# KAIST-AILab/SyncVSR

Hardware: AMD Instinct MI355X
Metric: lip-clips/sec training (29x88x88) (higher is better)
Workload: dtype bf16; 1 GPU; LRW training step (fwd+bwd+allreduce+clip+AdamW), ResNet18 + 6-layer 512-d encoder + vq audio-token CE head, random-init weights, N(0,1) clips 29x88x88, uniform tokens/labels; per_gpu_batch=32, global_batch=32, parallelism=dp1, hip_graph=False, enqueue=native step list

## Files before the change

include/syncvsr_hip.h:

```cpp
#ifndef SYNCVSR_HIP_H
#define SYNCVSR_HIP_H

#include <stdint.h>

#ifndef __HIP_PLATFORM_AMD__
typedef void* hipStream_t;
#else
#include <hip/hip_runtime_api.h>
#endif

#define SVSR_OK 0
#define SVSR_ERR_ARG 1001
#define SVSR_GRAD_ADD_DW 1
#define SVSR_GRAD_ADD_DB 2
#define SVSR_ERR_GROUP_OPEN 1003
#define SVSR_ERR_NO_GROUP 1004
#define SVSR_ERR_MASK_SIZE 1005

typedef struct svsr_wgrad_problem {
    const void* x; const void* dy; float* dw; float* dbias; const int* plan_dev; const int* meta;
    int Nimg; int in_pix; int Ci; int in_pitch; int Co; int out_pix; int out_pitch; int wt_taps;
} svsr_wgrad_problem;

typedef struct svsr_enc_layer {
// ... 27 lines not shown
int svsr_rows_plan(int Nimg, int P, int src0, int dst0, int Co_out, int* words, int cap_words, int* meta);
int svsr_igemm_fwd_kgroups(const int* meta, int Ci, int Co, int bn_epilogue);
int svsr_igemm_fwd(const void* in, const void* wt, void* out, void* out_pre, const float* bias, const void* addend, float* stats, const int* plan_dev, const int* meta, int Nimg, int in_pix, int Ci, int in_pitch, int Co, int out_pix, int out_pitch, int wt_taps, int act, int out_f32, float alpha, const unsigned* drop_seed, unsigned drop_site, float drop_p, hipStream_t stream);

int svsr_wgrad_plan(int Nimg, int H, int W, int Ci, int Co, int k, int stride, int pad, int* words, int cap_words, int* meta, int64_t* part_floats);
int svsr_wgrad_rows_plan(int Nimg, int P, int src0, int dst0, int Ci, int Co, int has_bias, int* words, int cap_words, int* meta, int64_t* part_floats);
int svsr_igemm_wgrad(const void* x, const void* dyp, float* dw, float* dbias, const int* plan_dev, const int* meta, int Nimg, int in_pix, int Ci, int in_pitch, int Co, int out_pix, int out_pitch, int wt_taps, float* part, int64_t part_floats, hipStream_t stream);
int svsr_wgrad_rows_plan_tile(int Nimg, int P, int src0, int dst0, int Ci, int Co, int has_bias, int bc, int* words, int cap_words, int* meta, int64_t* part_floats);
int64_t svsr_igemm_wgrad_group_bytes(int n);
int svsr_igemm_wgrad_group(const svsr_wgrad_problem* problems, int n, void* table_dev, int64_t table_bytes, hipStream_t stream);
int svsr_igemm_wgrad_v2(const void* x, const void* dyp, float* dw, float* dbias, const int* plan_dev, const int* meta, int Nimg, int in_pix, int Ci, int in_pitch, int Co, int out_pix, int out_pitch, int wt_taps, float* part, int64_t part_floats, int mode, hipStream_t stream);
int svsr_igemm_wgrad_group_v2(const svsr_wgrad_problem* problems, const int* modes, int n, void* table_dev, int64_t table_bytes, hipStream_t stream);

int svsr_conv3x3_c64_stat_rows(int Nimg, int H, int W);
int64_t svsr_conv3x3_c64_pixtab(int Nimg, int H, int W, int* out, int64_t cap);
int svsr_conv3x3_c64(const void* in, const void* wt, void* out, const void* addend, float* stats, int Nimg, int H, int W, const int* dy, const int* dx, const int* tw, const int* pixtab, hipStream_t stream);

int svsr_igemm_dgrad_bn(const void* in, const void* wt, void* out, const void* addend, float* stats, const int* plan_dev, const int* meta, int Nimg, int in_pix, int Ci, int in_pitch, int Co, int out_pix, int out_pitch, int wt_taps, const void* y, const void* x, const float* mean, const float* rstd, const float* gamma, const float* beta, int act, hipStream_t stream);
int svsr_igemm_dgrad_relu(const void* in, const void* wt, void* out, float* stats, const int* plan_dev, const int* meta, int Nimg, int in_pix, int Ci, int in_pitch, int Co, int out_pix, int out_pitch, int wt_taps, const void* y, const float* zeros, const float* ones, float gscale, hipStream_t stream);
int svsr_igemm_dgrad2(const void* in, const void* wt, const void* in2, const void* wt2, void* out, void* out_pre, const float* bias, float* stats, const int* plan_dev, const int* meta, int Nimg, int in_pix, int Ci, int in_pitch, int Co, int out_pix, int out_pitch, int wt_taps, int act, int out_f32, float alpha, const unsigned* drop_seed, unsigned drop_site, float drop_p, hipStream_t stream);
int svsr_igemm_dgrad2_bn(const void* in, const void* wt, const void* in2, const void* wt2, void* out, float* stats, const int* plan_dev, const int* meta, int Nimg, int in_pix, int Ci, int in_pitch, int Co, int out_pix, int out_pitch, int wt_taps, const void* y, const void* x, const float* mean, const float* rstd, const float* gamma, const float* beta, int act, hipStream_t stream);
int svsr_conv3x3_c64_dgrad_bn(const void* in, const void* wt, void* out, const void* addend, float* stats, int Nimg, int H, int W, const int* dy, const int* dx, const int* tw, const void* y, const void* x, const float* mean, const float* rstd, const float* gamma, const float* beta, int act, const int* pixtab, hipStream_t stream);
int svsr_bn_bwd_from_stats(const void* g, const void* x, const float* mean, const float* rstd, const float* gamma, const float* stats, int nrows, float* coef, float* dgamma, float* dbeta, void* dx, int64_t npix, int C, hipStream_t stream);


int svsr_conv3x3_wgrad_plan(int Nimg, int H, int W, int Ci, int Co, int* splits, int64_t* part_floats);
int svsr_conv3x3_wgrad(const void* x, const void* dy, float* dw, int Nimg, int H, int W, int Ci, int Co, float* part, int64_t part_floats, hipStream_t stream);
int svsr_conv3x3_wgrad_v2(const void* x, const void* dy, float* dw, int Nimg, int H, int W, int Ci, int Co, float* part, int64_t part_floats, int mode, hipStream_t stream);
int svsr_conv3x3_wgrad_chain(const void* x, const void* dy, float* dw, int Nimg, int H, int W, int Ci, int Co, float* part, int64_t part_floats, int mode, int defer, const float* pend_part, float* pend_dw, int pend_splits, int pend_Ci, int pend_Co, int pend_mode, hipStream_t stream);
int svsr_conv3x3_wgrad_reduce(const float* part, float* dw, int splits, int Ci, int Co, int mode, hipStream_t stream);

int svsr_stem_conv_fwd_stat_rows(int B, int T, int H, int W);
int64_t svsr_stem_conv_fwd_ws_bytes(int B, int T, int H, int W);
int svsr_stem_conv_fwd(const float* vid, const float* w, void* out, float* stats, int B, int T, int H, int W, void* ws, int64_t ws_bytes, hipStream_t stream);

int svsr_stem_conv_wgrad_plan(int B, int T, int H, int W, int* splits, int64_t* part_floats);
int svsr_stem_conv_wgrad(const float* vid, const void* dy, float* dw, int B, int T, int H, int W, int use_tr, float* part, int64_t part_floats, hipStream_t stream);

int svsr_stem_bwd_wgrad_ok(int B, int T, int H, int W);
int svsr_stem_bwd_wgrad(const float* vid, const void* gpool, const void* amax, const void* x, const float* mean, const float* rstd, const float* coef, float* dw, int B, int T, int H, int W, float* part, int64_t part_floats, hipStream_t stream);

int svsr_bn_finalize(const float* part, int nrows, int C, float count, float eps, float momentum, float* mean, float* rstd, float* running_mean, float* running_var, int64_t* num_batches_tracked, hipStream_t stream);

int svsr_bn_eval_prepare(const float* running_mean, const float* running_var, int C, float eps, float* mean, float* rstd, hipStream_t stream);

int svsr_bn_act_fwd(const void* x, const void* res, void* y, const float* mean, const float* rstd, const float* gamma, const float* beta, int64_t npix, int C, int act, hipStream_t stream);

int svsr_bn_act_bwd_rows(int64_t npix, int C);
int svsr_bn_act_bwd(const void* dy, const void* y, const void* x, const float* mean, const float* rstd, const float* gamma, float* slots, float* coef, float* dgamma, float* dbeta, void* dx, void* dres, int64_t npix, int C, int act, const float* beta, const void* res, hipStream_t stream);

int svsr_stem_bn_act_pool_fwd(const void* x, void* y, void* amax, const float* mean, const float* rstd, const float* gamma, const float* beta, int N, int Hc, int Wc, int Hp, int Wp, int C, int act, void* xwin, hipStream_t stream);

int svsr_stem_bn_act_pool_bwd_rows(int N, int Hc, int Wc, int C);
int svsr_stem_bn_act_pool_bwd(const void* dpool, const void* amax, const void* x, const float* mean, const float* rstd, const float* gamma, const float* beta, float* slots, float* coef, float* dgamma, float* dbeta, void* dx, int N, int Hc, int Wc, int Hp, int Wp, int C, int act, const void* xwin, void* gpool, hipStream_t stream);

int svsr_avgpool_fwd(const void* x, void* y, int64_t N, int HW, int C, hipStream_t stream);
int svsr_avgpool_bwd(const void* dy, void* dx, int64_t N, int HW, int C, hipStream_t stream);

int svsr_add_ln_fwd(const void* a, const void* r, const float* gamma, const float* beta, void* y, float* mean, float* rstd, int R, int D, float eps, hipStream_t stream);
int svsr_add_ln_bwd_rows(int R);
int svsr_add_ln_bwd(const void* dy, const void* a, const void* r, const float* gamma, const float* mean, const float* rstd, void* ds, float* dgamma, float* dbeta, int R, int D, const void* addend, float* part, hipStream_t stream);
int svsr_add_ln_bwd_partials(const void* dy, const void* a, const void* r, const float* gamma, const float* mean, const float* rstd, void* ds, int R, int D, const void* addend, float* part, hipStream_t stream);
int svsr_add_ln_bwd_branch(const void* dy, const void* a, const void* r, const float* gamma, const float* mean, const float* rstd, void* ds, int R, int D, const void* addend, float* part, void* ds2, float alpha2, const unsigned* drop_seed, unsigned drop_site, float drop_p, hipStream_t stream);
int svsr_bias_act_bwd_partials(const void* dy, const void* z, void* dz, float* db, int R, int N, int n_valid, int ld, int act, float gscale, float* part, hipStream_t stream);

int svsr_embed_ln_fwd(const void* feats, const float* cls, const float* pos, const float* type0, const float* gamma, const float* beta, void* sum_out, void* y, float* mean, float* rstd, int B, int S, int D, float eps, const unsigned* drop_seed, unsigned site_in, float p_in, unsigned site_out, float p_out, hipStream_t stream);
int svsr_embed_bwd_scatter(const void* ds, void* dfeats, float* dcls, float* dpos, float* dtype0, int B, int S, int D, float* part, const unsigned* drop_seed, unsigned site_in, float p_in, hipStream_t stream);

int svsr_rmsnorm_fwd(const void* x, const float* g, void* y, float* inv, int R, int D, int ld, float eps, hipStream_t stream);
// ... 175 lines not shown
```

syncvsr_amd/csrc/norm_act.hip:

```cpp
#include "common.h"

#define BNF_CL 4
#define BNF_RL 64
__device__ __forceinline__ void bn_rows_sum(const float* __restrict__ part, int nrows, int C, int c, bool live, int rl, int cl,
                                            double (*sred)[2][BNF_CL], double& s, double& q) {
    double a = 0.0, b = 0.0;
    if (live) {
        int r = rl;
        for (; r + 7 * BNF_RL < nrows; r += 8 * BNF_RL) {
            float av[8], bv[8];
#pragma unroll
            for (int k = 0; k < 8; ++k) {
                av[k] = part[((long)(r + k * BNF_RL) * 2 + 0) * C + c];
                bv[k] = part[((long)(r + k * BNF_RL) * 2 + 1) * C + c];
            }
#pragma unroll
            for (int k = 0; k < 8; ++k) { a += (double)av[k]; b += (double)bv[k]; }
        }
        for (; r + 3 * BNF_RL < nrows; r += 4 * BNF_RL) {
            const float a0 = part[((long)r * 2 + 0) * C + c], b0 = part[((long)r * 2 + 1) * C + c];
            const float a1 = part[((long)(r + BNF_RL) * 2 + 0) * C + c], b1 = part[((long)(r + BNF_RL) * 2 + 1) * C + c];
            const float a2 = part[((long)(r + 2 * BNF_RL) * 2 + 0) * C + c], b2 = part[((long)(r + 2 * BNF_RL) * 2 + 1) * C + c];
            const float a3 = part[((long)(r + 3 * BNF_RL) * 2 + 0) * C + c], b3 = part[((long)(r + 3 * BNF_RL) * 2 + 1) * C + c];
            a = (((a + (double)a0) + (double)a1) + (double)a2) + (double)a3;
// ... 56 lines not shown
    }
    for (; idx < nvec; idx += stride) {
        float f[8];
        unpack8(reinterpret_cast<const u32x4*>(x)[idx], f);
#pragma unroll
        for (int k = 0; k < 8; ++k) f[k] = __builtin_fmaf(f[k], sc[k], sh[k]);
        if (res != nullptr) {
            float r[8];
            unpack8(reinterpret_cast<const u32x4*>(res)[idx], r);
#pragma unroll
            for (int k = 0; k < 8; ++k) f[k] += r[k];
        }
        if (act == 1) {
#pragma unroll
            for (int k = 0; k < 8; ++k) f[k] = fmaxf(f[k], 0.f);
        } else if (act == 2) {
#pragma unroll
            for (int k = 0; k < 8; ++k) f[k] = swish(f[k]);
        }
        reinterpret_cast<u32x4*>(y)[idx] = pack8(f);
    }
}

__device__ __forceinline__ void reduce_to_row(float* sred, const float* s1, const float* s2, int cv, int C, float* part,
                                              int first_group = 0) {
    const int tid = threadIdx.x;
#pragma unroll
    for (int k = 0; k < 8; ++k) { sred[tid * 16 + k] = s1[k]; sred[tid * 16 + 8 + k] = s2[k]; }
    __syncthreads();
    const long row = (long)blockIdx.y * gridDim.x + blockIdx.x;
    for (int o = tid; o < cv * 16; o += 256) {
        const int g = o >> 4, k = o & 15;
        float acc = 0.f;
        int t0 = g - first_group;
        if (t0 < 0) t0 += cv;
        for (int t = t0; t < 256; t += cv) acc += sred[t * 16 + k];
        const int which = k >> 3, c = g * 8 + (k & 7);
        part[(row * 2 + which) * C + c] = acc;
    }
}

template <int act>
__global__ __launch_bounds__(256) void k_bn_act_bwd_reduce(const bf16_t* __restrict__ dy, const bf16_t* __restrict__ y,
                                                           const bf16_t* __restrict__ x, const float* __restrict__ mean,
                                                           const float* __restrict__ rstd, long nvec, int C,
                                                           float* slots, const float* __restrict__ gamma,
// ... 70 lines not shown
    }
    for (; idx < nvec; idx += stride) {
        float g[8], xv[8], o[8];
        unpack8(reinterpret_cast<const u32x4*>(dy)[idx], g);
        unpack8(reinterpret_cast<const u32x4*>(x)[idx], xv);
        if (act == 1) {
            float yv[8];
            unpack8(reinterpret_cast<const u32x4*>(y)[idx], yv);
#pragma unroll
            for (int k = 0; k < 8; ++k) g[k] = yv[k] > 0.f ? g[k] : 0.f;
        } else if (act == 2) {
            float rv[8];
#pragma unroll
            for (int k = 0; k < 8; ++k) rv[k] = 0.f;
            if (res != nullptr) unpack8(reinterpret_cast<const u32x4*>(res)[idx], rv);
#pragma unroll
            for (int k = 0; k < 8; ++k) g[k] *= swish_grad((xv[k] - mu[k]) * rs[k] * ga[k] + be[k] + rv[k]);
        }
#pragma unroll
        for (int k = 0; k < 8; ++k) o[k] = k0[k] * (g[k] - k1[k] - (xv[k] - mu[k]) * rs[k] * k2[k]);
        reinterpret_cast<u32x4*>(dx)[idx] = pack8(o);
        if (dres != nullptr) reinterpret_cast<u32x4*>(dres)[idx] = pack8(g);
    }
}

struct StemRowIter {
    int W, cv, cshift, rpb;
    float inv_wcv;
    __device__ __forceinline__ void decode(int e, int& rl, int& w, int& c8) const {
        const int wcv = W << cshift;
        rl = (int)((float)e * inv_wcv);
        int rem = e - rl * wcv;
        if (rem < 0) { rl--; rem += wcv; } else if (rem >= wcv) { rl++; rem -= wcv; }
        w = rem >> cshift;
        c8 = rem & (cv - 1);
    }
};

template <int ACT>
__global__ __launch_bounds__(256) void k_stem_bn_act_pool_fwd(const bf16_t* __restrict__ x, bf16_t* __restrict__ y,
                                                               unsigned char* __restrict__ amax, bf16_t* __restrict__ xwin,
                                                               const float* __restrict__ mean, const float* __restrict__ rstd,
                                                               const float* __restrict__ gamma, const float* __restrict__ beta,
                                                               int N, int Hc, int Wc, int Hp, int Wp, int C, StemRowIter it) {
    const int n = blockIdx.y, row0 = blockIdx.x * it.rpb;
    const int c0 = (threadIdx.x & (it.cv - 1)) * 8;
// ... 417 lines not shown
int svsr_bn_finalize(const float* part, int nrows, int C, float count, float eps, float momentum, float* mean, float* rstd,
                     float* running_mean, float* running_var, int64_t* num_batches_tracked, hipStream_t stream) {
    if (nrows < 1 || C < 1) return SVSR_ERR_ARG;
    hipLaunchKernelGGL(k_bn_finalize, dim3((C + BNF_CL - 1) / BNF_CL), dim3(BNF_CL * BNF_RL), 0, stream, part, nrows, C, count, eps, momentum, mean, rstd,
                       running_mean, running_var, (long*)num_batches_tracked);
    return svsr_check_launch();
}

int svsr_bn_eval_prepare(const float* running_mean, const float* running_var, int C, float eps, float* mean, float* rstd,
                         hipStream_t stream) {
    hipLaunchKernelGGL(k_bn_eval_prepare, dim3((C + 127) / 128), dim3(128), 0, stream, running_mean, running_var, C, eps, mean, rstd);
    return svsr_check_launch();
}

int svsr_bn_act_fwd(const void* x, const void* res, void* y, const float* mean, const float* rstd, const float* gamma,
                    const float* beta, int64_t npix, int C, int act, hipStream_t stream) {
    if (!chan_ok_any(C)) return SVSR_ERR_ARG;
    const long nvec = npix * (C / 8);
    hipLaunchKernelGGL(k_bn_act_fwd, dim3(ew_grid_for(nvec, C)), dim3(256), 0, stream, (const bf16_t*)x, (const bf16_t*)res, (bf16_t*)y,
                       mean, rstd, gamma, beta, nvec, C, act);
    return svsr_check_launch();
}

int svsr_bn_act_bwd_rows(int64_t npix, int C) { return chan_ok_any(C) && npix > 0 ? bn_bwd_grid(npix * (C / 8), C) : 0; }

int svsr_bn_act_bwd(const void* dy, const void* y, const void* x, const float* mean, const float* rstd, const float* gamma,
                    float* slots, float* coef, float* dgamma, float* dbeta, void* dx, void* dres, int64_t npix, int C, int act,
                    const float* beta, const void* res, hipStream_t stream) {
    if (!chan_ok_any(C)) return SVSR_ERR_ARG;
    if (act == 2 && beta == nullptr) return SVSR_ERR_ARG;
    const long nvec = npix * (C / 8);
    const int grid = bn_bwd_grid(nvec, C);
    const int grid_apply = ew_grid_for(nvec, C);
#define SVSR_BN_BWD_REDUCE(A) hipLaunchKernelGGL(k_bn_act_bwd_reduce<A>, dim3(grid), dim3(256), 0, stream, (const bf16_t*)dy, (const bf16_t*)y, \
                       (const bf16_t*)x, mean, rstd, nvec, C, slots, gamma, beta, (const bf16_t*)res)
#define SVSR_BN_BWD_APPLY(A) hipLaunchKernelGGL(k_bn_act_bwd_apply<A>, dim3(grid_apply), dim3(256), 0, stream, (const bf16_t*)dy, (const bf16_t*)y, \
                       (const bf16_t*)x, mean, rstd, coef, (bf16_t*)dx, (bf16_t*)dres, nvec, C, gamma, beta, (const bf16_t*)res)
    if (act < 0 || act > 2) return SVSR_ERR_ARG;
    if (act == 2) SVSR_BN_BWD_REDUCE(2); else if (act == 1) SVSR_BN_BWD_REDUCE(1); else SVSR_BN_BWD_REDUCE(0);
    hipLaunchKernelGGL(k_bn_bwd_finalize, dim3((C + BNF_CL - 1) / BNF_CL), dim3(BNF_CL * BNF_RL), 0, stream, slots, grid, C, (float)npix, gamma, rstd, dgamma, dbeta, coef);
    if (act == 2) SVSR_BN_BWD_APPLY(2); else if (act == 1) SVSR_BN_BWD_APPLY(1); else SVSR_BN_BWD_APPLY(0);
    return svsr_check_launch();
}

int svsr_bn_bwd_from_stats(const void* g, const void* x, const float* mean, const float* rstd, const float* gamma, const float* stats,
                           int nrows, float* coef, float* dgamma, float* dbeta, void* dx, int64_t npix, int C, hipStream_t stream) {
    if (!chan_ok_any(C) || nrows < 1 || npix < 1 || g == nullptr || x == nullptr || stats == nullptr || dx == nullptr) return SVSR_ERR_ARG;
    const long nvec = npix * (C / 8);
    hipLaunchKernelGGL(k_bn_bwd_finalize, dim3((C + BNF_CL - 1) / BNF_CL), dim3(BNF_CL * BNF_RL), 0, stream, stats, nrows, C, (float)npix, gamma, rstd, dgamma, dbeta, coef);
    hipLaunchKernelGGL(k_bn_act_bwd_apply<0>, dim3(ew_grid_for(nvec, C)), dim3(256), 0, stream, (const bf16_t*)g, (const bf16_t*)nullptr,
                       (const bf16_t*)x, mean, rstd, coef, (bf16_t*)dx, (bf16_t*)nullptr, nvec, C, gamma, (const float*)nullptr, (const bf16_t*)nullptr);
    return svsr_check_launch();
}

int svsr_stem_bn_act_pool_fwd(const void* x, void* y, void* amax, const float* mean, const float* rstd, const float* gamma,
                              const float* beta, int N, int Hc, int Wc, int Hp, int Wp, int C, int act, void* xwin, hipStream_t stream) {
    if (!chan_ok(C) || (act != SVSR_ACT_GELU && act != SVSR_ACT_SWISH)) return SVSR_ERR_ARG;
    if (N < 1 || Hc < 1 || Wc < 1 || Hp != (Hc - 1) / 2 + 1 || Wp != (Wc - 1) / 2 + 1) return SVSR_ERR_ARG;
    StemRowIter it;
    if (!stem_iter(it, C, Wp, Hp)) return SVSR_ERR_ARG;
    const dim3 grid((Hp + it.rpb - 1) / it.rpb, N);
    if (act == SVSR_ACT_SWISH)
        hipLaunchKernelGGL(k_stem_bn_act_pool_fwd<2>, grid, dim3(256), 0, stream, (const bf16_t*)x, (bf16_t*)y, (unsigned char*)amax, (bf16_t*)xwin, mean,
                           rstd, gamma, beta, N, Hc, Wc, Hp, Wp, C, it);
    else
        hipLaunchKernelGGL(k_stem_bn_act_pool_fwd<1>, grid, dim3(256), 0, stream, (const bf16_t*)x, (bf16_t*)y, (unsigned char*)amax, (bf16_t*)xwin, mean,
                           rstd, gamma, beta, N, Hc, Wc, Hp, Wp, C, it);
    return svsr_check_launch();
}

static inline bool stem_bwd_uses_lds(int Wp, int C) { return (size_t)(STEM_BR / 2 + 1) * Wp * C * 3 <= 60 * 1024; }
static inline size_t stem_gather_lds(int Wc) { const size_t t = (size_t)(((2 * STEM_GP + 1) * Wc * 8 + 255) / 256 * 256) * 16; return t > 16384 ? t : 16384; }
static inline bool stem_bwd_gathers(int Wc, int Wp, int C) { return C == 64 && stem_bwd_uses_lds(Wp, C) && stem_gather_lds(Wc) <= 64 * 1024; }

// ... 91 lines not shown
```

syncvsr_amd/csrc/steplist.hip:

```cpp
#include <stdlib.h>
#include <string.h>

#include <string>
#include <unordered_map>
#include <utility>
#include <vector>

#include "common.h"
#include "../../include/syncvsr_hip.h"

namespace {

typedef int64_t Slot;

template <typename T> struct FromSlot;
template <> struct FromSlot<int> { static int get(Slot s) { return (int)s; } };
template <> struct FromSlot<unsigned> { static unsigned get(Slot s) { return (unsigned)s; } };
template <> struct FromSlot<int64_t> { static int64_t get(Slot s) { return s; } };
template <> struct FromSlot<float> { static float get(Slot s) { double d; memcpy(&d, &s, sizeof d); return (float)d; } };
template <typename P> struct FromSlot<P*> { static P* get(Slot s) { return reinterpret_cast<P*>((uintptr_t)s); } };

template <typename... A, size_t... I>
int invoke(int (*fn)(A...), const Slot* s, std::index_sequence<I...>) { return fn(FromSlot<A>::get(s[I])...); }

template <typename... A>
int thunk_n(int (*)(A...)) { return (int)sizeof...(A); }

typedef int (*Thunk)(const Slot*);
struct Entry { Thunk call; int nargs; };

template <typename F, F fn> struct Bind;
template <typename... A, int (*fn)(A...)>
struct Bind<int (*)(A...), fn> {
    static int call(const Slot* s) { return invoke(fn, s, std::index_sequence_for<A...>{}); }
    static constexpr int nargs = (int)sizeof...(A);
};

#define SVSR_REG(f) {#f, Entry{&Bind<decltype(&f), &f>::call, Bind<decltype(&f), &f>::nargs}}

const std::unordered_map<std::string, Entry>& registry() {
    static const std::unordered_map<std::string, Entry> r = {
        SVSR_REG(svsr_colsum_rows), SVSR_REG(svsr_colsum_rows_multi), SVSR_REG(svsr_igemm_fwd), SVSR_REG(svsr_igemm_wgrad), SVSR_REG(svsr_conv3x3_c64),
        SVSR_REG(svsr_igemm_dgrad_bn), SVSR_REG(svsr_igemm_dgrad_relu), SVSR_REG(svsr_igemm_dgrad2), SVSR_REG(svsr_igemm_dgrad2_bn), SVSR_REG(svsr_conv3x3_c64_dgrad_bn), SVSR_REG(svsr_bn_bwd_from_stats),
        SVSR_REG(svsr_conv3x3_wgrad), SVSR_REG(svsr_stem_conv_fwd), SVSR_REG(svsr_stem_conv_wgrad), SVSR_REG(svsr_stem_bwd_wgrad), SVSR_REG(svsr_bn_finalize),
        SVSR_REG(svsr_bn_eval_prepare), SVSR_REG(svsr_bn_act_fwd), SVSR_REG(svsr_bn_act_bwd), SVSR_REG(svsr_stem_bn_act_pool_fwd),
        SVSR_REG(svsr_stem_bn_act_pool_bwd), SVSR_REG(svsr_avgpool_fwd), SVSR_REG(svsr_avgpool_bwd), SVSR_REG(svsr_add_ln_fwd),
        SVSR_REG(svsr_add_ln_bwd), SVSR_REG(svsr_embed_ln_fwd), SVSR_REG(svsr_embed_bwd_scatter), SVSR_REG(svsr_rmsnorm_fwd),
        SVSR_REG(svsr_rmsnorm_bwd), SVSR_REG(svsr_rotary), SVSR_REG(svsr_geglu_fwd), SVSR_REG(svsr_geglu_bwd), SVSR_REG(svsr_xt_embed_fwd),
        SVSR_REG(svsr_xt_embed_bwd), SVSR_REG(svsr_bias_act_bwd), SVSR_REG(svsr_ce_fwd), SVSR_REG(svsr_ce_bwd), SVSR_REG(svsr_linear_ce_fwd), SVSR_REG(svsr_linear_ce_bwd), SVSR_REG(svsr_topk_acc),
        SVSR_REG(svsr_grad_sumsq), SVSR_REG(svsr_grad_sumsq_parts), SVSR_REG(svsr_adamw_step), SVSR_REG(svsr_adamw_range), SVSR_REG(svsr_adamw_onecycle_step), SVSR_REG(svsr_adamw_onecycle_range), SVSR_REG(svsr_cast_bf16), SVSR_REG(svsr_transpose_cast_multi),
        SVSR_REG(svsr_transpose_bf16_multi), SVSR_REG(svsr_fill_f32), SVSR_REG(svsr_clip_prep), SVSR_REG(svsr_mha_fwd), SVSR_REG(svsr_mha_bwd), SVSR_REG(svsr_mha_flash_fwd), SVSR_REG(svsr_mha_flash_bwd), SVSR_REG(svsr_mha_flash_bwd_parts), SVSR_REG(svsr_mha_pe_transpose),
        SVSR_REG(svsr_glu_dwconv_fwd), SVSR_REG(svsr_glu_dwconv_bwd), SVSR_REG(svsr_glu_dwconv_bwd_parts), SVSR_REG(svsr_ctc_fwd), SVSR_REG(svsr_ctc_grad),
        SVSR_REG(svsr_ctc_prefix_score), SVSR_REG(svsr_lrs_targets), SVSR_REG(svsr_embed_pos_fwd), SVSR_REG(svsr_embed_pos_bwd), SVSR_REG(svsr_ls_loss_fwd),
        SVSR_REG(svsr_ls_loss_bwd), SVSR_REG(svsr_scale_bf16), SVSR_REG(svsr_word_add), SVSR_REG(svsr_lincomb2), SVSR_REG(svsr_igemm_wgrad_group), SVSR_REG(svsr_enc_fwd), SVSR_REG(svsr_enc_bwd), SVSR_REG(svsr_lincomb3_ratio), SVSR_REG(svsr_add_ln_bwd_partials), SVSR_REG(svsr_add_ln_bwd_branch), SVSR_REG(svsr_bias_act_bwd_partials),
        SVSR_REG(svsr_memcpy_async), SVSR_REG(svsr_w2v_conv0), SVSR_REG(svsr_w2v_norm_gelu), SVSR_REG(svsr_w2v_quantize),
        SVSR_REG(svsr_igemm_wgrad_v2), SVSR_REG(svsr_igemm_wgrad_group_v2), SVSR_REG(svsr_conv3x3_wgrad_v2), SVSR_REG(svsr_fill_ranges),
        SVSR_REG(svsr_conv3x3_wgrad_chain), SVSR_REG(svsr_conv3x3_wgrad_reduce),
        SVSR_REG(svsr_mha_table_fwd), SVSR_REG(svsr_lm_embed_fwd),
        SVSR_REG(svsr_beam_select), SVSR_REG(svsr_ctc_prefix_score_clips), SVSR_REG(svsr_mha_src_step_fwd), SVSR_REG(svsr_ctc_align),
        SVSR_REG(svsr_ctc_frame_best), SVSR_REG(svsr_ctc_collapse), SVSR_REG(svsr_edit_distance),
        SVSR_REG(svsr_tconv_fwd), SVSR_REG(svsr_tcn_se_fwd), SVSR_REG(svsr_tcn_norm_pool_fwd),
        SVSR_REG(svsr_tconv_fwd_save), SVSR_REG(svsr_tconv_epi_bwd), SVSR_REG(svsr_tconv_dgrad), SVSR_REG(svsr_tconv_wgrad), SVSR_REG(svsr_tcn_se_bwd),
        SVSR_REG(svsr_tcn_norm_pool_bwd), SVSR_REG(svsr_tcn_fold),
        SVSR_REG(svsr_tconv_fwd_ext), SVSR_REG(svsr_tcn_colstats), SVSR_REG(svsr_tconv_apply), SVSR_REG(svsr_tconv_epi_bwd_bs), SVSR_REG(svsr_tconv_bn_bwd),
        SVSR_REG(svsr_tconv_dgrad_ext), SVSR_REG(svsr_tconv_wgrad_ext), SVSR_REG(svsr_tcn_norm_pool_bwd_bs),
        SVSR_REG(svsr_lrs_clip_prep), SVSR_REG(svsr_wave_prep),
        SVSR_REG(svsr_lrw_clip_sums), SVSR_REG(svsr_lrw_clip_mix),
        SVSR_REG(svsr_dctcn_clip_sums), SVSR_REG(svsr_dctcn_clip_mix), SVSR_REG(svsr_dctcn_wave_trim),
// ... 259 lines not shown
```

syncvsr_amd/model.py:

```python
from __future__ import annotations

import math
from typing import Any, Optional

import torch
import torch.nn as nn

from . import ops
from .config import Config, audio_codec_dims
from .init import buffer_specs, hidden_dim, init_state_dict, pad64, param_specs, phys_shape, resnet_block_specs, xt_dims

BF16 = torch.bfloat16


class _SideStream:

    def __init__(self) -> None:
        self.stream: Optional[torch.cuda.Stream] = None
        self.keep: list = []
        self._issuing = False
        self.enabled = False
        self.enabled_small = False

    def run(self, fn, *keep, small: bool = False, behind_main: bool = True) -> None:
# ... 613 lines not shown


def _bn_stats(st: _ParamStore, base: str, training: bool, count: int, stats):
    ws = st.bn[base]
    if training:
        ops.bn_finalize(stats, ws["mean"].numel(), count, ws["mean"], ws["rstd"], st.buffers[f"{base}.running_mean"],
                        st.buffers[f"{base}.running_var"], st.buffers[f"{base}.num_batches_tracked"])
    else:
        ops.bn_eval_prepare(st.buffers[f"{base}.running_mean"], st.buffers[f"{base}.running_var"], ws["mean"], ws["rstd"])
    return ws["mean"], ws["rstd"]


def _conv_bn(st: _ParamStore, tape: dict, x: torch.Tensor, conv: str, bn: str, k: int, stride: int, pad: int, training: bool,
             res: Optional[torch.Tensor], act: int) -> torch.Tensor:
    o, n, shape = st.offsets[f"{conv}.weight"]
    w16 = st.w16[o : o + n].view(shape[0], k, k, shape[1])
    c, stats = ops.conv2d_fwd(x, w16, k, stride, pad, want_stats=training)
    mean, rstd = _bn_stats(st, bn, training, c.numel() // c.shape[-1], stats)
    y = ops.bn_act_fwd(c, res, mean, rstd, st.p32(f"{bn}.weight"), st.p32(f"{bn}.bias"), act)
    tape[conv] = dict(x=x, c=c, y=y, mean=mean, rstd=rstd, k=k, stride=stride, pad=pad, act=act, bn=bn, res=res)
    return y


def _trunk_blocks(model):
    for prefix, inp, planes, stride, down in resnet_block_specs():
        yield model.trunk_name + prefix[len("resnet"):], inp, planes, stride, down


def _frontend_forward(model, st: "_ParamStore", tape: dict, videos: torch.Tensor, training: bool) -> torch.Tensor:
    B, _, T, H, W = videos.shape
    N = B * T
    sc, sb, act = model.stem_name + ".0", model.stem_name + ".1", model.trunk_act
    c, stats = ops.stem_conv_fwd(videos, st.p32(f"{sc}.weight"), want_stats=training)
    mean, rstd = _bn_stats(st, sb, training, c.numel() // 64, stats)
    if training:
        x, amax, xwin = ops.stem_bn_gelu_pool_fwd(c, mean, rstd, st.p32(f"{sb}.weight"), st.p32(f"{sb}.bias"), model.stem_act, want_win=True)
    else:
        (x, amax), xwin = ops.stem_bn_gelu_pool_fwd(c, mean, rstd, st.p32(f"{sb}.weight"), st.p32(f"{sb}.bias"), model.stem_act), None
    tape["stem"] = dict(videos=videos, c=c, amax=amax, xwin=xwin, mean=mean, rstd=rstd, pooled_shape=tuple(x.shape))
    for prefix, inp, planes, stride, down in _trunk_blocks(model):
        xin = x
        if down and training and model._side.enabled:
            box: dict = {}
            model._side.run(lambda xin=xin, prefix=prefix, stride=stride: box.__setitem__(
                "idt", _conv_bn(st, tape, xin, f"{prefix}.downsample.0", f"{prefix}.downsample.1", 1, stride, 0, training, None, 0)), xin)
            o1 = _conv_bn(st, tape, xin, f"{prefix}.conv1", f"{prefix}.bn1", 3, stride, 1, training, None, act)
            model._side.join()
            idt = box["idt"]
        else:
            o1 = _conv_bn(st, tape, xin, f"{prefix}.conv1", f"{prefix}.bn1", 3, stride, 1, training, None, act)
            idt = _conv_bn(st, tape, xin, f"{prefix}.downsample.0", f"{prefix}.downsample.1", 1, stride, 0, training, None, 0) if down else xin
        x = _conv_bn(st, tape, o1, f"{prefix}.conv2", f"{prefix}.bn2", 3, 1, 1, training, idt, act)
    tape["trunk_out_shape"] = tuple(x.shape)
    return ops.avgpool_fwd(x)


def _frontend_backward(model, st: "_ParamStore", tape: dict, dfeats: torch.Tensor) -> None:
    act = model.trunk_act
    dx = ops.avgpool_bwd(dfeats, tape["trunk_out_shape"])
    fused = act in (1, 2) and ops.BN_BWD_FUSED
    dx_stats = None
    blocks = list(_trunk_blocks(model))
    rec = tape.get("_record_grads")
    for bi in range(len(blocks) - 1, -1, -1):
        prefix, inp, planes, stride, down = blocks[bi]
        if rec is not None:
            rec[prefix] = (dx.clone(), dx_stats is not None)
        t2 = tape[f"{prefix}.conv2"]
        ws2 = st.bn[t2["bn"]]
        if dx_stats is not None:
            dres = dx
            dc2 = ops.bn_bwd_from_stats(dx, t2["c"], t2["mean"], t2["rstd"], st.p32(f"{t2['bn']}.weight"), dx_stats, ws2["coef"],
                                        st.g32(f"{t2['bn']}.weight"), st.g32(f"{t2['bn']}.bias"))
        else:
            dc2, dres = ops.bn_act_bwd(dx, t2["y"], t2["c"], t2["mean"], t2["rstd"], st.p32(f"{t2['bn']}.weight"), ws2["coef"],
                                       st.g32(f"{t2['bn']}.weight"), st.g32(f"{t2['bn']}.bias"), act, True,
                                       beta=st.p32(f"{t2['bn']}.bias"), res=t2["res"])
        _conv_wgrad(model, st, f"{prefix}.conv2", t2, dc2)
        t1 = tape[f"{prefix}.conv1"]
        ws1 = st.bn[t1["bn"]]
        w2t = st.t16(f"{prefix}.conv2.weight").view(planes, 3, 3, planes)
        if fused:
            g1, st1 = ops.conv2d_dgrad_bn(dc2, w2t, 3, 1, 1, t2["x"].shape[1:3], None, None, t1["c"], t1["mean"], t1["rstd"],
                                          st.p32(f"{t1['bn']}.weight"), st.p32(f"{t1['bn']}.bias"), act)
            dc1 = ops.bn_bwd_from_stats(g1, t1["c"], t1["mean"], t1["rstd"], st.p32(f"{t1['bn']}.weight"), st1, ws1["coef"],
                                        st.g32(f"{t1['bn']}.weight"), st.g32(f"{t1['bn']}.bias"))
        else:
            do1 = ops.conv2d_dgrad(dc2, w2t, 3, 1, 1, t2["x"].shape[1:3])
            dc1, _ = ops.bn_act_bwd(do1, t1["y"], t1["c"], t1["mean"], t1["rstd"], st.p32(f"{t1['bn']}.weight"), ws1["coef"],
                                    st.g32(f"{t1['bn']}.weight"), st.g32(f"{t1['bn']}.bias"), act, False, beta=st.p32(f"{t1['bn']}.bias"))
        _conv_wgrad(model, st, f"{prefix}.conv1", t1, dc1)
        in_hw = t1["x"].shape[1:3]
        w1t = st.t16(f"{prefix}.conv1.weight").view(inp, 3, 3, planes)
        tp = tape[f"{blocks[bi - 1][0]}.conv2"] if fused and bi > 0 else None
        if tp is not None:
            tp_aux = tp["y"] if act == 1 else tp["res"]
            tp_gb = (st.p32(f"{tp['bn']}.weight"), st.p32(f"{tp['bn']}.bias"), act)
        if down:
            td = tape[f"{prefix}.downsample.0"]
            wsd = st.bn[td["bn"]]
            dcd, _ = ops.bn_act_bwd(dres, None, td["c"], td["mean"], td["rstd"], st.p32(f"{td['bn']}.weight"), wsd["coef"],
                                    st.g32(f"{td['bn']}.weight"), st.g32(f"{td['bn']}.bias"), 0, False)
            _conv_wgrad(model, st, f"{prefix}.downsample.0", td, dcd)
            wdt = st.t16(f"{prefix}.downsample.0.weight").view(inp, 1, 1, planes)
            if ops.DGRAD2 and stride == 2:
                if tp is not None:
                    dx, dx_stats = ops.conv2d_dgrad2(dc1, w1t, dcd, wdt, in_hw, bn=(tp_aux, tp["c"], tp["mean"], tp["rstd"], *tp_gb))
                else:
                    dx, dx_stats = ops.conv2d_dgrad2(dc1, w1t, dcd, wdt, in_hw), None
            else:
                dxd = ops.conv2d_dgrad(dcd, wdt, 1, stride, 0, in_hw)
                if tp is not None:
                    dx, dx_stats = ops.conv2d_dgrad_bn(dc1, w1t, 3, stride, 1, in_hw, dxd, tp_aux, tp["c"], tp["mean"], tp["rstd"], *tp_gb)
                else:
                    dx, dx_stats = ops.conv2d_dgrad(dc1, w1t, 3, stride, 1, in_hw, addend=dxd), None
        elif tp is not None:
            dx, dx_stats = ops.conv2d_dgrad_bn(dc1, w1t, 3, stride, 1, in_hw, dres, tp_aux, tp["c"], tp["mean"], tp["rstd"], *tp_gb)
        else:
            dx, dx_stats = ops.conv2d_dgrad(dc1, w1t, 3, stride, 1, in_hw, addend=dres), None
        _ready(model, st, f"{prefix}.conv1.weight")
    _flush_w3_chain(model)
    ts = tape["stem"]
    if rec is not None:
        rec["stem"] = (dx.clone(), False)
    sc, sb = model.stem_name + ".0", model.stem_name + ".1"
# ... 513 lines not shown
```

syncvsr_amd/ops.py:

```python
from __future__ import annotations

import bisect
import ctypes
import os
import struct
from contextlib import contextmanager, nullcontext
from collections import namedtuple
from typing import Callable, Optional, Sequence

import torch

from . import _lib

BF16 = torch.bfloat16
BN_EPS = 1e-5
BN_MOMENTUM = 0.1
HALO_WGRAD = True


_DEV_INDEX: Optional[int] = None
STREAM_OVERRIDE: Optional[int] = None


def _stream() -> int:
# ... 789 lines not shown
        _call("svsr_igemm_dgrad2", *head, None, None, None, plan.words.data_ptr(), plan.meta, N, Ho * Wo, Co, Co, Ci, H * W, Ci, 9, 0, 0, 1.0,
              *_drop(None), _stream(), label=label, flops=flops)
        return dx
    y, x, mean, rstd, gamma, beta, act = bn
    if x.shape != dx.shape or not x.is_contiguous() or (y is not None and (y.shape != x.shape or not y.is_contiguous())):
        raise ValueError("conv2d_dgrad2: y / x must be contiguous tensors with the geometry of the result")
    if (y is None or act == 2) and (gamma is None or beta is None):
        raise ValueError("conv2d_dgrad2: y=None / act=2 need gamma and beta")
    stats = scratch(plan.tiles * 2 * Ci)
    _call("svsr_igemm_dgrad2_bn", *head, _p(stats), plan.words.data_ptr(), plan.meta, N, Ho * Wo, Co, Co, Ci, H * W, Ci, 9, _p(y), _p(x),
          _p(mean), _p(rstd), _p(gamma), _p(beta), act, _stream(), label=label + "+bn", flops=flops)
    return dx, (stats, plan.tiles)


def bn_bwd_from_stats(g, x, mean, rstd, gamma, stats, coef, dgamma, dbeta) -> torch.Tensor:
    part, rows = stats
    C = x.shape[-1]
    dx = torch.empty_like(x)
    _call("svsr_bn_bwd_from_stats", _p(g), _p(x), _p(mean), _p(rstd), _p(gamma), _p(part), rows, _p(coef), _p(dgamma), _p(dbeta), _p(dx),
          x.numel() // C, C, _stream())
    return dx


def conv2d_wgrad(x: torch.Tensor, dy: torch.Tensor, dw: torch.Tensor, k: int, stride: int, pad: int, use_tr: bool = True, mode: Optional[int] = None) -> None:
    N, H, W, Ci = x.shape
    _, Ho, Wo, Co = dy.shape
    if HALO_WGRAD and use_tr and k == 3 and stride == 1 and pad == 1 and W <= 29 and H * W >= 100 and Ci % 64 == 0 and Co % 64 == 0:
        _, nfl = _query("svsr_conv3x3_wgrad_plan", N, H, W, Ci, Co)
        part = scratch(nfl) if nfl else None
        _call("svsr_conv3x3_wgrad_v2", _p(x), _p(dy), _p(dw), N, H, W, Ci, Co, _p(part), nfl, _grad_add(dw, Co * 9 * Ci) if mode is None else mode & 1, _stream(),
              label="k_wgrad3x3_halo", flops=2.0 * N * H * W * Co * Ci * 9)
        return
    igemm_wgrad(wgrad_conv_plan(N, H, W, Ci, Co, k, stride, pad), x, dy, dw, Nimg=N, in_pix=H * W, Ci=Ci, in_pitch=Ci, Co=Co,
                out_pix=Ho * Wo, out_pitch=Co, wt_taps=k * k, flops=2.0 * N * Ho * Wo * Co * Ci * k * k, mode=mode)


def halo_wgrad_ok(x: torch.Tensor, dy: torch.Tensor, k: int, stride: int, pad: int) -> bool:
    N, H, W, Ci = x.shape
    Co = dy.shape[-1]
    return HALO_WGRAD and k == 3 and stride == 1 and pad == 1 and W <= 29 and H * W >= 100 and Ci % 64 == 0 and Co % 64 == 0


_W3_SETS: dict[tuple, torch.Tensor] = {}


def _w3_set(which: int, nfloats: int) -> torch.Tensor:
# ... 187 lines not shown


def stem_bwd_wgrad(videos: torch.Tensor, gpool, amax, x, mean, rstd, coef, dw: torch.Tensor) -> None:
    B, _, T, H, W = videos.shape
    _, nfl = _query("svsr_stem_conv_wgrad_plan", B, T, H, W)
    _call("svsr_stem_bwd_wgrad", _p(videos), _p(gpool), _p(amax), _p(x), _p(mean), _p(rstd), _p(coef), _p(dw), B, T, H, W, _p(scratch(nfl)), nfl,
          _stream(), label="k_stem_bwd_wgrad", flops=2.0 * B * T * (H // 2) * (W // 2) * 64 * 245)


def bn_finalize(stats, C: int, count: int, mean, rstd, running_mean=None, running_var=None, nbt=None) -> None:
    part, rows = stats
    _call("svsr_bn_finalize", _p(part), rows, C, float(count), BN_EPS, BN_MOMENTUM, _p(mean), _p(rstd), _p(running_mean), _p(running_var),
          _p(nbt), _stream())


def bn_eval_prepare(running_mean, running_var, mean, rstd) -> None:
    _call("svsr_bn_eval_prepare", _p(running_mean), _p(running_var), running_mean.numel(), BN_EPS, _p(mean), _p(rstd), _stream())


def bn_act_fwd(x, res, mean, rstd, gamma, beta, act: int) -> torch.Tensor:
    C = x.shape[-1]
    y = torch.empty_like(x)
    _call("svsr_bn_act_fwd", _p(x), _p(res), _p(y), _p(mean), _p(rstd), _p(gamma), _p(beta), x.numel() // C, C, act, _stream())
    return y


def bn_act_bwd(dy, y, x, mean, rstd, gamma, coef, dgamma, dbeta, act: int, want_dres: bool, beta=None, res=None):
    C = x.shape[-1]
    dx = torch.empty_like(x)
    dres = torch.empty_like(x) if want_dres else None
    slots = scratch(_query("svsr_bn_act_bwd_rows", x.numel() // C, C)[0] * 2 * C)
    _call("svsr_bn_act_bwd", _p(dy), _p(y), _p(x), _p(mean), _p(rstd), _p(gamma), _p(slots), _p(coef), _p(dgamma), _p(dbeta), _p(dx),
          _p(dres), x.numel() // C, C, act, _p(beta), _p(res), _stream())
    return dx, dres


def avgpool_fwd(x: torch.Tensor) -> torch.Tensor:
    N, H, W, C = x.shape
    y = torch.empty((N, C), dtype=BF16, device=x.device)
    _call("svsr_avgpool_fwd", _p(x), _p(y), N, H * W, C, _stream())
    return y


def avgpool_bwd(dy: torch.Tensor, shape) -> torch.Tensor:
    N, H, W, C = shape
    dx = torch.empty(shape, dtype=BF16, device=dy.device)
# ... 1398 lines not shown
```

Measured before the change: 7095 clips/s.

## Fuse downsample BN into residual BN-add-ReLU and its backward reduction

In ResNet downsample blocks the downsample branch now stores only its conv output and stats. The downsample BN is applied inside a new dual-BN add+ReLU kernel for the block's conv2, so the separate downsample bn_act_fwd pass and its materialised output are no longer needed. In backward, the conv2 BN apply kernel also accumulates the downsample BN reduction sums, so the downsample branch can use bn_bwd_from_stats instead of a full bn_act_bwd reduction pass. The cost is an extra tensor read in each fused kernel. The downsample branch is also now joined just before conv2's epilogue rather than earlier, so the side stream overlaps with conv1.

```diff
diff --git a/include/syncvsr_hip.h b/include/syncvsr_hip.h
--- a/include/syncvsr_hip.h
+++ b/include/syncvsr_hip.h
@@ -73,6 +73,7 @@
 int svsr_igemm_dgrad2_bn(const void* in, const void* wt, const void* in2, const void* wt2, void* out, float* stats, const int* plan_dev, const int* meta, int Nimg, int in_pix, int Ci, int in_pitch, int Co, int out_pix, int out_pitch, int wt_taps, const void* y, const void* x, const float* mean, const float* rstd, const float* gamma, const float* beta, int act, hipStream_t stream);
 int svsr_conv3x3_c64_dgrad_bn(const void* in, const void* wt, void* out, const void* addend, float* stats, int Nimg, int H, int W, const int* dy, const int* dx, const int* tw, const void* y, const void* x, const float* mean, const float* rstd, const float* gamma, const float* beta, int act, const int* pixtab, hipStream_t stream);
 int svsr_bn_bwd_from_stats(const void* g, const void* x, const float* mean, const float* rstd, const float* gamma, const float* stats, int nrows, float* coef, float* dgamma, float* dbeta, void* dx, int64_t npix, int C, hipStream_t stream);
+int svsr_bn_bwd_from_stats_ds(const void* g, const void* x, const float* mean, const float* rstd, const float* gamma, const float* stats, int nrows, float* coef, float* dgamma, float* dbeta, void* dx, const void* xd, const float* mean_d, const float* rstd_d, float* rows_d, int64_t npix, int C, hipStream_t stream);
 
 
 int svsr_conv3x3_wgrad_plan(int Nimg, int H, int W, int Ci, int Co, int* splits, int64_t* part_floats);
@@ -96,6 +97,7 @@
 int svsr_bn_eval_prepare(const float* running_mean, const float* running_var, int C, float eps, float* mean, float* rstd, hipStream_t stream);
 
 int svsr_bn_act_fwd(const void* x, const void* res, void* y, const float* mean, const float* rstd, const float* gamma, const float* beta, int64_t npix, int C, int act, hipStream_t stream);
+int svsr_bn_act_fwd2(const void* x, const void* xd, void* y, const float* mean, const float* rstd, const float* gamma, const float* beta, const float* mean_d, const float* rstd_d, const float* gamma_d, const float* beta_d, int64_t npix, int C, hipStream_t stream);
 
 int svsr_bn_act_bwd_rows(int64_t npix, int C);
 int svsr_bn_act_bwd(const void* dy, const void* y, const void* x, const float* mean, const float* rstd, const float* gamma, float* slots, float* coef, float* dgamma, float* dbeta, void* dx, void* dres, int64_t npix, int C, int act, const float* beta, const void* res, hipStream_t stream);
diff --git a/syncvsr_amd/csrc/norm_act.hip b/syncvsr_amd/csrc/norm_act.hip
--- a/syncvsr_amd/csrc/norm_act.hip
+++ b/syncvsr_amd/csrc/norm_act.hip
@@ -102,6 +102,37 @@
     }
 }
 
+__global__ __launch_bounds__(256) void k_bn_act_fwd2(const bf16_t* __restrict__ x, const bf16_t* __restrict__ xd, bf16_t* __restrict__ y,
+                                                     const float* __restrict__ mean, const float* __restrict__ rstd,
+                                                     const float* __restrict__ gamma, const float* __restrict__ beta,
+                                                     const float* __restrict__ mean_d, const float* __restrict__ rstd_d,
+                                                     const float* __restrict__ gamma_d, const float* __restrict__ beta_d, long nvec, int C) {
+    const int cv = C >> 3;
+    long idx = (long)blockIdx.x * 256 + threadIdx.x;
+    const long stride = (long)gridDim.x * 256;
+    if (idx >= nvec) return;
+    const int c0 = (int)(idx % cv) * 8;
+    float sc[8], sh[8], scd[8], shd[8];
+#pragma unroll
+    for (int k = 0; k < 8; ++k) {
+        sc[k] = gamma[c0 + k] * rstd[c0 + k];
+        sh[k] = __builtin_fmaf(-mean[c0 + k], sc[k], beta[c0 + k]);
+        scd[k] = gamma_d[c0 + k] * rstd_d[c0 + k];
+        shd[k] = __builtin_fmaf(-mean_d[c0 + k], scd[k], beta_d[c0 + k]);
+    }
+    for (; idx < nvec; idx += stride) {
+        float f[8], d[8], r[8];
+        unpack8(reinterpret_cast<const u32x4*>(x)[idx], f);
+        unpack8(reinterpret_cast<const u32x4*>(xd)[idx], d);
+#pragma unroll
+        for (int k = 0; k < 8; ++k) { f[k] = __builtin_fmaf(f[k], sc[k], sh[k]); d[k] = __builtin_fmaf(d[k], scd[k], shd[k]); }
+        unpack8(pack8(d), r);
+#pragma unroll
+        for (int k = 0; k < 8; ++k) f[k] = fmaxf(f[k] + r[k], 0.f);
+        reinterpret_cast<u32x4*>(y)[idx] = pack8(f);
+    }
+}
+
 __device__ __forceinline__ void reduce_to_row(float* sred, const float* s1, const float* s2, int cv, int C, float* part,
                                               int first_group = 0) {
     const int tid = threadIdx.x;
@@ -218,6 +249,38 @@
         reinterpret_cast<u32x4*>(dx)[idx] = pack8(o);
         if (dres != nullptr) reinterpret_cast<u32x4*>(dres)[idx] = pack8(g);
     }
+}
+
+__global__ __launch_bounds__(256) void k_bn_bwd_apply_ds(const bf16_t* __restrict__ dy, const bf16_t* __restrict__ x,
+                                                         const float* __restrict__ mean, const float* __restrict__ rstd,
+                                                         const float* __restrict__ coef, bf16_t* __restrict__ dx,
+                                                         const bf16_t* __restrict__ xd, const float* __restrict__ mean_d,
+                                                         const float* __restrict__ rstd_d, float* slots_d, long nvec, int C) {
+    __shared__ float sred[256 * 16];
+    const int cv = C >> 3;
+    long idx = (long)blockIdx.x * 256 + threadIdx.x;
+    const long stride = (long)gridDim.x * 256;
+    const int c0 = (int)(idx % cv) * 8;
+    const int first_group = (int)(((long)blockIdx.x * 256) % cv);
+    float mu[8], rs[8], k0[8], k1[8], k2[8], mud[8], rsd[8], s1[8], s2[8];
+#pragma unroll
+    for (int k = 0; k < 8; ++k) {
+        mu[k] = mean[c0 + k]; rs[k] = rstd[c0 + k];
+        k0[k] = coef[c0 + k]; k1[k] = coef[C + c0 + k]; k2[k] = coef[2 * C + c0 + k];
+        mud[k] = mean_d[c0 + k]; rsd[k] = rstd_d[c0 + k]; s1[k] = 0.f; s2[k] = 0.f;
+    }
+    for (; idx < nvec; idx += stride) {
+        float g[8], xv[8], xdv[8], o[8];
+        unpack8(reinterpret_cast<const u32x4*>(dy)[idx], g);
+        unpack8(reinterpret_cast<const u32x4*>(x)[idx], xv);
+        unpack8(reinterpret_cast<const u32x4*>(xd)[idx], xdv);
+#pragma unroll
+        for (int k = 0; k < 8; ++k) o[k] = k0[k] * (g[k] - k1[k] - (xv[k] - mu[k]) * rs[k] * k2[k]);
+        reinterpret_cast<u32x4*>(dx)[idx] = pack8(o);
+#pragma unroll
+        for (int k = 0; k < 8; ++k) { s1[k] += g[k]; s2[k] += g[k] * (xdv[k] - mud[k]) * rsd[k]; }
+    }
+    reduce_to_row(sred, s1, s2, cv, C, slots_d, first_group);
 }
 
 struct StemRowIter {
@@ -681,6 +744,15 @@
     return svsr_check_launch();
 }
 
+int svsr_bn_act_fwd2(const void* x, const void* xd, void* y, const float* mean, const float* rstd, const float* gamma, const float* beta,
+                     const float* mean_d, const float* rstd_d, const float* gamma_d, const float* beta_d, int64_t npix, int C, hipStream_t stream) {
+    if (!chan_ok_any(C) || npix < 1 || x == nullptr || xd == nullptr || y == nullptr) return SVSR_ERR_ARG;
+    const long nvec = npix * (C / 8);
+    hipLaunchKernelGGL(k_bn_act_fwd2, dim3(ew_grid_for(nvec, C)), dim3(256), 0, stream, (const bf16_t*)x, (const bf16_t*)xd, (bf16_t*)y,
+                       mean, rstd, gamma, beta, mean_d, rstd_d, gamma_d, beta_d, nvec, C);
+    return svsr_check_launch();
+}
+
 int svsr_bn_act_bwd_rows(int64_t npix, int C) { return chan_ok_any(C) && npix > 0 ? bn_bwd_grid(npix * (C / 8), C) : 0; }
 
 int svsr_bn_act_bwd(const void* dy, const void* y, const void* x, const float* mean, const float* rstd, const float* gamma,
@@ -709,6 +781,18 @@
     hipLaunchKernelGGL(k_bn_bwd_finalize, dim3((C + BNF_CL - 1) / BNF_CL), dim3(BNF_CL * BNF_RL), 0, stream, stats, nrows, C, (float)npix, gamma, rstd, dgamma, dbeta, coef);
     hipLaunchKernelGGL(k_bn_act_bwd_apply<0>, dim3(ew_grid_for(nvec, C)), dim3(256), 0, stream, (const bf16_t*)g, (const bf16_t*)nullptr,
                        (const bf16_t*)x, mean, rstd, coef, (bf16_t*)dx, (bf16_t*)nullptr, nvec, C, gamma, (const float*)nullptr, (const bf16_t*)nullptr);
+    return svsr_check_launch();
+}
+
+int svsr_bn_bwd_from_stats_ds(const void* g, const void* x, const float* mean, const float* rstd, const float* gamma, const float* stats,
+                              int nrows, float* coef, float* dgamma, float* dbeta, void* dx, const void* xd, const float* mean_d,
+                              const float* rstd_d, float* rows_d, int64_t npix, int C, hipStream_t stream) {
+    if (!chan_ok_any(C) || nrows < 1 || npix < 1 || g == nullptr || x == nullptr || stats == nullptr || dx == nullptr) return SVSR_ERR_ARG;
+    if (xd == nullptr || mean_d == nullptr || rstd_d == nullptr || rows_d == nullptr) return SVSR_ERR_ARG;
+    const long nvec = npix * (C / 8);
+    hipLaunchKernelGGL(k_bn_bwd_finalize, dim3((C + BNF_CL - 1) / BNF_CL), dim3(BNF_CL * BNF_RL), 0, stream, stats, nrows, C, (float)npix, gamma, rstd, dgamma, dbeta, coef);
+    hipLaunchKernelGGL(k_bn_bwd_apply_ds, dim3(bn_bwd_grid(nvec, C)), dim3(256), 0, stream, (const bf16_t*)g, (const bf16_t*)x, mean, rstd, coef,
+                       (bf16_t*)dx, (const bf16_t*)xd, mean_d, rstd_d, rows_d, nvec, C);
     return svsr_check_launch();
 }
 
diff --git a/syncvsr_amd/csrc/steplist.hip b/syncvsr_amd/csrc/steplist.hip
--- a/syncvsr_amd/csrc/steplist.hip
+++ b/syncvsr_amd/csrc/steplist.hip
@@ -41,9 +41,9 @@
 const std::unordered_map<std::string, Entry>& registry() {
     static const std::unordered_map<std::string, Entry> r = {
         SVSR_REG(svsr_colsum_rows), SVSR_REG(svsr_colsum_rows_multi), SVSR_REG(svsr_igemm_fwd), SVSR_REG(svsr_igemm_wgrad), SVSR_REG(svsr_conv3x3_c64),
-        SVSR_REG(svsr_igemm_dgrad_bn), SVSR_REG(svsr_igemm_dgrad_relu), SVSR_REG(svsr_igemm_dgrad2), SVSR_REG(svsr_igemm_dgrad2_bn), SVSR_REG(svsr_conv3x3_c64_dgrad_bn), SVSR_REG(svsr_bn_bwd_from_stats),
+        SVSR_REG(svsr_igemm_dgrad_bn), SVSR_REG(svsr_igemm_dgrad_relu), SVSR_REG(svsr_igemm_dgrad2), SVSR_REG(svsr_igemm_dgrad2_bn), SVSR_REG(svsr_conv3x3_c64_dgrad_bn), SVSR_REG(svsr_bn_bwd_from_stats), SVSR_REG(svsr_bn_bwd_from_stats_ds),
         SVSR_REG(svsr_conv3x3_wgrad), SVSR_REG(svsr_stem_conv_fwd), SVSR_REG(svsr_stem_conv_wgrad), SVSR_REG(svsr_stem_bwd_wgrad), SVSR_REG(svsr_bn_finalize),
-        SVSR_REG(svsr_bn_eval_prepare), SVSR_REG(svsr_bn_act_fwd), SVSR_REG(svsr_bn_act_bwd), SVSR_REG(svsr_stem_bn_act_pool_fwd),
+        SVSR_REG(svsr_bn_eval_prepare), SVSR_REG(svsr_bn_act_fwd), SVSR_REG(svsr_bn_act_fwd2), SVSR_REG(svsr_bn_act_bwd), SVSR_REG(svsr_stem_bn_act_pool_fwd),
         SVSR_REG(svsr_stem_bn_act_pool_bwd), SVSR_REG(svsr_avgpool_fwd), SVSR_REG(svsr_avgpool_bwd), SVSR_REG(svsr_add_ln_fwd),
         SVSR_REG(svsr_add_ln_bwd), SVSR_REG(svsr_embed_ln_fwd), SVSR_REG(svsr_embed_bwd_scatter), SVSR_REG(svsr_rmsnorm_fwd),
         SVSR_REG(svsr_rmsnorm_bwd), SVSR_REG(svsr_rotary), SVSR_REG(svsr_geglu_fwd), SVSR_REG(svsr_geglu_bwd), SVSR_REG(svsr_xt_embed_fwd),
diff --git a/syncvsr_amd/model.py b/syncvsr_amd/model.py
--- a/syncvsr_amd/model.py
+++ b/syncvsr_amd/model.py
@@ -659,6 +659,27 @@
     return y
 
 
+def _conv_stats(st: _ParamStore, tape: dict, x: torch.Tensor, conv: str, bn: str, k: int, stride: int, pad: int) -> dict:
+    o, n, shape = st.offsets[f"{conv}.weight"]
+    w16 = st.w16[o : o + n].view(shape[0], k, k, shape[1])
+    c, stats = ops.conv2d_fwd(x, w16, k, stride, pad, want_stats=True)
+    mean, rstd = _bn_stats(st, bn, True, c.numel() // c.shape[-1], stats)
+    tape[conv] = dict(x=x, c=c, y=None, mean=mean, rstd=rstd, k=k, stride=stride, pad=pad, act=0, bn=bn, res=None)
+    return tape[conv]
+
+
+def _conv_bn2(st: _ParamStore, tape: dict, x: torch.Tensor, conv: str, bn: str, get_td) -> torch.Tensor:
+    o, n, shape = st.offsets[f"{conv}.weight"]
+    w16 = st.w16[o : o + n].view(shape[0], 3, 3, shape[1])
+    c, stats = ops.conv2d_fwd(x, w16, 3, 1, 1, want_stats=True)
+    mean, rstd = _bn_stats(st, bn, True, c.numel() // c.shape[-1], stats)
+    td = get_td()
+    y = ops.bn_act_fwd2(c, td["c"], mean, rstd, st.p32(f"{bn}.weight"), st.p32(f"{bn}.bias"), td["mean"], td["rstd"],
+                        st.p32(f"{td['bn']}.weight"), st.p32(f"{td['bn']}.bias"))
+    tape[conv] = dict(x=x, c=c, y=y, mean=mean, rstd=rstd, k=3, stride=1, pad=1, act=1, bn=bn, res=None)
+    return y
+
+
 def _trunk_blocks(model):
     for prefix, inp, planes, stride, down in resnet_block_specs():
         yield model.trunk_name + prefix[len("resnet"):], inp, planes, stride, down
@@ -677,6 +698,16 @@
     tape["stem"] = dict(videos=videos, c=c, amax=amax, xwin=xwin, mean=mean, rstd=rstd, pooled_shape=tuple(x.shape))
     for prefix, inp, planes, stride, down in _trunk_blocks(model):
         xin = x
+        if down and training and act == 1:
+            dn, db = f"{prefix}.downsample.0", f"{prefix}.downsample.1"
+            model._side.run(lambda xin=xin, dn=dn, db=db, stride=stride: _conv_stats(st, tape, xin, dn, db, 1, stride, 0), xin)
+            o1 = _conv_bn(st, tape, xin, f"{prefix}.conv1", f"{prefix}.bn1", 3, stride, 1, training, None, act)
+
+            def joined(dn=dn):
+                model._side.join()
+                return tape[dn]
+            x = _conv_bn2(st, tape, o1, f"{prefix}.conv2", f"{prefix}.bn2", joined)
+            continue
         if down and training and model._side.enabled:
             box: dict = {}
             model._side.run(lambda xin=xin, prefix=prefix, stride=stride: box.__setitem__(
@@ -705,7 +736,14 @@
             rec[prefix] = (dx.clone(), dx_stats is not None)
         t2 = tape[f"{prefix}.conv2"]
         ws2 = st.bn[t2["bn"]]
-        if dx_stats is not None:
+        dcd = None
+        if dx_stats is not None and down and act == 1:
+            dres, td = dx, tape[f"{prefix}.downsample.0"]
+            dc2, d_stats = ops.bn_bwd_from_stats_ds(dx, t2["c"], t2["mean"], t2["rstd"], st.p32(f"{t2['bn']}.weight"), dx_stats, ws2["coef"],
+                                                    st.g32(f"{t2['bn']}.weight"), st.g32(f"{t2['bn']}.bias"), td["c"], td["mean"], td["rstd"])
+            dcd = ops.bn_bwd_from_stats(dres, td["c"], td["mean"], td["rstd"], st.p32(f"{td['bn']}.weight"), d_stats, st.bn[td["bn"]]["coef"],
+                                        st.g32(f"{td['bn']}.weight"), st.g32(f"{td['bn']}.bias"))
+        elif dx_stats is not None:
             dres = dx
             dc2 = ops.bn_bwd_from_stats(dx, t2["c"], t2["mean"], t2["rstd"], st.p32(f"{t2['bn']}.weight"), dx_stats, ws2["coef"],
                                         st.g32(f"{t2['bn']}.weight"), st.g32(f"{t2['bn']}.bias"))
@@ -736,8 +774,9 @@
         if down:
             td = tape[f"{prefix}.downsample.0"]
             wsd = st.bn[td["bn"]]
-            dcd, _ = ops.bn_act_bwd(dres, None, td["c"], td["mean"], td["rstd"], st.p32(f"{td['bn']}.weight"), wsd["coef"],
-                                    st.g32(f"{td['bn']}.weight"), st.g32(f"{td['bn']}.bias"), 0, False)
+            if dcd is None:
+                dcd, _ = ops.bn_act_bwd(dres, None, td["c"], td["mean"], td["rstd"], st.p32(f"{td['bn']}.weight"), wsd["coef"],
+                                        st.g32(f"{td['bn']}.weight"), st.g32(f"{td['bn']}.bias"), 0, False)
             _conv_wgrad(model, st, f"{prefix}.downsample.0", td, dcd)
             wdt = st.t16(f"{prefix}.downsample.0.weight").view(inp, 1, 1, planes)
             if ops.DGRAD2 and stride == 2:
diff --git a/syncvsr_amd/ops.py b/syncvsr_amd/ops.py
--- a/syncvsr_amd/ops.py
+++ b/syncvsr_amd/ops.py
@@ -835,6 +835,17 @@
     return dx
 
 
+def bn_bwd_from_stats_ds(g, x, mean, rstd, gamma, stats, coef, dgamma, dbeta, xd, mean_d, rstd_d):
+    part, rows = stats
+    C = x.shape[-1]
+    dx = torch.empty_like(x)
+    rows_d = _query("svsr_bn_act_bwd_rows", x.numel() // C, C)[0]
+    slots = scratch(rows_d * 2 * C)
+    _call("svsr_bn_bwd_from_stats_ds", _p(g), _p(x), _p(mean), _p(rstd), _p(gamma), _p(part), rows, _p(coef), _p(dgamma), _p(dbeta), _p(dx),
+          _p(xd), _p(mean_d), _p(rstd_d), _p(slots), x.numel() // C, C, _stream())
+    return dx, (slots, rows_d)
+
+
 def conv2d_wgrad(x: torch.Tensor, dy: torch.Tensor, dw: torch.Tensor, k: int, stride: int, pad: int, use_tr: bool = True, mode: Optional[int] = None) -> None:
     N, H, W, Ci = x.shape
     _, Ho, Wo, Co = dy.shape
@@ -1068,6 +1079,14 @@
     C = x.shape[-1]
     y = torch.empty_like(x)
     _call("svsr_bn_act_fwd", _p(x), _p(res), _p(y), _p(mean), _p(rstd), _p(gamma), _p(beta), x.numel() // C, C, act, _stream())
+    return y
+
+
+def bn_act_fwd2(x, xd, mean, rstd, gamma, beta, mean_d, rstd_d, gamma_d, beta_d) -> torch.Tensor:
+    C = x.shape[-1]
+    y = torch.empty_like(x)
+    _call("svsr_bn_act_fwd2", _p(x), _p(xd), _p(y), _p(mean), _p(rstd), _p(gamma), _p(beta), _p(mean_d), _p(rstd_d), _p(gamma_d), _p(beta_d),
+          x.numel() // C, C, _stream())
     return y
 
 
```

Result: faster. 7174 clips/s (median of 6 runs) (+1.1%).
